# deepinv/deepinv

Hardware: AMD Instinct MI355X
Metric: PnP-PGD slices/sec (50 iters), 2D MRI 8-coil 320x320, 4x radial mask, DRUNet (higher is better)
Workload: dtype f32: fp32 multiplies and accumulation on the fp32 matrix cores (v_mfma_f32_32x32x2_f32); ResBlock convs as Winograd F(4x4,3x3), U = G g G^T formed in fp64 and rounded once; the three 2x2 stride-2 down convolutions (2 % of the FLOPs) as an exact three-part bf16 operand split with six products and fp3

## Files before the change

### deepinv_amd/csrc/drunet_bf16s.hip

```cpp
#include "drunet_common.hpp"

using namespace dinv;
using namespace dinv_drunet;

namespace {

__device__ __forceinline__ unsigned f2bf(float f) {
#ifdef DINV_EMU
    unsigned u = __float_as_uint(f);
    if ((u & 0x7fffffffu) > 0x7f800000u) return (u >> 16) | 0x40u;
    u += 0x7fffu + ((u >> 16) & 1u);
    return u >> 16;
#else
    return (unsigned)__builtin_bit_cast(unsigned short, (__bf16)f);
#endif
}
__device__ __forceinline__ float bf2f(unsigned h) { return __uint_as_float(h << 16); }

__device__ __forceinline__ void split8(const float4& a, const float4& b, uint4& hi, uint4& lo) {
    const float v[8] = {a.x, a.y, a.z, a.w, b.x, b.y, b.z, b.w};
    unsigned h[8], l[8];
#pragma unroll
    for (int e = 0; e < 8; ++e) {
        h[e] = f2bf(v[e]);
        l[e] = f2bf(v[e] - bf2f(h[e]));
    }
    hi = make_uint4(h[0] | (h[1] << 16), h[2] | (h[3] << 16), h[4] | (h[5] << 16), h[6] | (h[7] << 16));
    lo = make_uint4(l[0] | (l[1] << 16), l[2] | (l[3] << 16), l[4] | (l[5] << 16), l[6] | (l[7] << 16));
}

__device__ __forceinline__ void split8x3(const float4& a, const float4& b, uint4& hi, uint4& mi, uint4& lo) {
    const float v[8] = {a.x, a.y, a.z, a.w, b.x, b.y, b.z, b.w};
    unsigned h[8], m[8], l[8];
#pragma unroll
    for (int e = 0; e < 8; ++e) {
        h[e] = f2bf(v[e]);
        const float r1 = v[e] - bf2f(h[e]);
        m[e] = f2bf(r1);
        l[e] = f2bf(r1 - bf2f(m[e]));
    }
    hi = make_uint4(h[0] | (h[1] << 16), h[2] | (h[3] << 16), h[4] | (h[5] << 16), h[6] | (h[7] << 16));
    mi = make_uint4(m[0] | (m[1] << 16), m[2] | (m[3] << 16), m[4] | (m[5] << 16), m[6] | (m[7] << 16));
    lo = make_uint4(l[0] | (l[1] << 16), l[2] | (l[3] << 16), l[4] | (l[5] << 16), l[6] | (l[7] << 16));
}

#ifdef DINV_EMU
__device__ __forceinline__ f32x16 mfma_bf16(const uint4& a, const uint4& b, const f32x16& c) {
    emu_bf16x8 av, bv;
    std::memcpy(&av, &a, 16);
    std::memcpy(&bv, &b, 16);
    return emu_mfma_f32_32x32x16_bf16(av, bv, c);
}
#else
typedef __bf16 bf16x8 __attribute__((ext_vector_type(8)));
__device__ __forceinline__ f32x16 mfma_bf16(const uint4& a, const uint4& b, const f32x16& c) {
    return __builtin_amdgcn_mfma_f32_32x32x16_bf16(__builtin_bit_cast(bf16x8, a), __builtin_bit_cast(bf16x8, b), c, 0, 0, 0);
}
#endif

struct DownSArgs {
    Geom gi, go;
    const float* x;
    const uint4* w;
    float* y;
    int32_t cin, cout;
    int64_t ntiles, per_xcd;
    DepthMap dm;
};

template <bool ACC, int NPL>
__global__ __launch_bounds__(256) void down2x2_bf16s_kernel(DownSArgs a) {
    constexpr int WU = NPL * 128;
    constexpr int WPT = (WU + 255) / 256;
    __shared__ uint4 wl[2][WU];
    const int tid = threadIdx.x, lane = tid & 63, wv = tid >> 6;
    const int l31 = lane & 31, lhi = lane >> 5;
    const int64_t logical = (int64_t)(blockIdx.x & 7) * a.per_xcd + (blockIdx.x >> 3);
    if (logical >= a.ntiles) return;
    const int nct = a.cout / 64;
    const int64_t q0 = (logical / nct) * 256 + wv * 64;
    const int co0 = (int)(logical % nct) * 64;
    int64_t ioff[2];
    bool in[2];
#pragma unroll
    for (int n = 0; n < 2; ++n) {
        const int64_t q = q0 + n * 32 + l31;
        in[n] = interior(a.go, q);
        ioff[n] = a.gi.sl;
        if (in[n]) {
            const int64_t b = q / a.go.plane;
            const int64_t bi = depth_pair(a.dm, b);
            if (bi < 0) in[n] = false;
            else {
                const int qi = (int)(q - b * a.go.plane);
                const int R = qi / a.go.wp, C = qi - R * a.go.wp;
                ioff[n] = a.gi.sl + bi * a.gi.plane + (int64_t)(2 * (R - 1) + 1) * a.gi.wp + (2 * (C - 1) + 1);
            }
        }
    }
    f32x16 acc[2][2];
#pragma unroll
    for (int m = 0; m < 2; ++m)
#pragma unroll
        for (int n = 0; n < 2; ++n)
#pragma unroll
            for (int r = 0; r < 16; ++r) acc[m][n][r] = 0.f;
    const int S = a.cin / 16, nsteps = 4 * S;
    float4 ba[2], bb[2];
    uint4 wreg[WPT];
    auto issue = [&](int g) {
        const int tap = g / S, s = g - tap * S;
        const int64_t toff = (int64_t)(tap >> 1) * a.gi.wp + (tap & 1);
#pragma unroll
        for (int k = 0; k < WPT; ++k) {
            const int u = tid + 256 * k;
            if (u < WU) wreg[k] = a.w[((int64_t)g * (2 * NPL) + (u >> 6)) * a.cout + co0 + (u & 63)];
        }
#pragma unroll
        for (int n = 0; n < 2; ++n) {
            const float* xb = a.x + ((int64_t)(2 * s + lhi) * a.gi.cs + ioff[n] + toff) * 8;
            ba[n] = ld4(xb);
            bb[n] = ld4(xb + 4);
        }
    };
    uint4 Bp[NPL][2];
    auto commit = [&](int stage) {
#pragma unroll
        for (int k = 0; k < WPT; ++k)
            if (tid + 256 * k < WU) wl[stage][tid + 256 * k] = wreg[k];
#pragma unroll
        for (int n = 0; n < 2; ++n) {
            if constexpr (NPL == 2) split8(ba[n], bb[n], Bp[0][n], Bp[1][n]);
            else split8x3(ba[n], bb[n], Bp[0][n], Bp[1][n], Bp[2][n]);
        }
    };
    issue(0);
    commit(0);
    if (nsteps > 1) issue(1);
    __syncthreads();
    constexpr int NPROD = NPL == 2 ? 3 : 6;
    constexpr int PA[6] = {0, 1, 0, 0, 1, 0}, PB2[3] = {1, 0, 0};
    constexpr int QA[6] = {1, 0, 2, 0, 1, 0}, QB[6] = {1, 2, 0, 1, 0, 0};
    for (int g = 0; g < nsteps; ++g) {
        const uint4* ws = wl[g & 1];
        uint4 A[NPL][2];
#pragma unroll
        for (int pl = 0; pl < NPL; ++pl)
#pragma unroll
            for (int m = 0; m < 2; ++m) A[pl][m] = ws[pl * 128 + lhi * 64 + m * 32 + l31];
#pragma unroll
        for (int e = 0; e < NPROD; ++e) {
            const int pa = NPL == 2 ? PA[e] : QA[e], pb = NPL == 2 ? PB2[e] : QB[e];
#pragma unroll
            for (int m = 0; m < 2; ++m)
#pragma unroll
                for (int n = 0; n < 2; ++n) acc[m][n] = mfma_bf16(A[pa][m], Bp[pb][n], acc[m][n]);
        }
        if (g + 1 < nsteps) {
            commit((g + 1) & 1);
            if (g + 2 < nsteps) issue(g + 2);
        }
        lds_barrier();
    }
#pragma unroll
    for (int n = 0; n < 2; ++n) {
        const int64_t q = q0 + n * 32 + l31;
        if (q >= a.go.np) continue;
        store_tile<2, false, ACC ? 1 : 0>(acc, n, a.go.sl + q, in[n], co0 / 8, a.cout / 8, a.go.cs, lhi, a.y, ACC ? a.y : nullptr,
                                          nullptr);
    }
}

struct UpSArgs {
    Geom gi, go;
    const float* x;
    const float* x2;
    const uint4* w;
    float* y;
    int32_t cin, cout;
    DepthMap dm;
};

#ifdef DINV_EMU
#define DINV_BF16S_UP_ATTR
#else
#define DINV_BF16S_UP_ATTR __attribute__((amdgpu_waves_per_eu(2, 2)))
#endif
template <bool SKIP>
__global__ __launch_bounds__(256) DINV_BF16S_UP_ATTR void up2x2_bf16s_kernel(UpSArgs a) {
    __shared__ uint4 wl[2][1024];
    const int tid = threadIdx.x, lane = tid & 63, wv = tid >> 6;
    const int l31 = lane & 31, lhi = lane >> 5;
    const int tp = wv & 1, pg = wv >> 1;
    const int co0 = blockIdx.y * 64;
    const int64_t p0 = (int64_t)blockIdx.x * 128 + pg * 64;
    int64_t ioff[2], ooff[2];
    bool in[2];
#pragma unroll
    for (int n = 0; n < 2; ++n) {
        const int64_t p = p0 + n * 32 + l31;
        in[n] = interior(a.gi, p);
        ioff[n] = a.gi.sl + (in[n] ? p : 0);
        ooff[n] = 0;
        if (in[n]) {
            const int64_t b = p / a.gi.plane;
            const int64_t bo = depth_pair(a.dm, b);
            if (bo < 0) in[n] = false;
            else {
                const int pi = (int)(p - b * a.gi.plane);
                const int r = pi / a.gi.wp, c = pi - r * a.gi.wp;
                ooff[n] = a.go.sl + bo * a.go.plane + (int64_t)(2 * (r - 1) + 1 + tp) * a.go.wp + (2 * (c - 1) + 1);
            }
        }
    }
    f32x16 acc[2][2][2];
#pragma unroll
    for (int t = 0; t < 2; ++t)
#pragma unroll
        for (int m = 0; m < 2; ++m)
#pragma unroll
            for (int n = 0; n < 2; ++n)
#pragma unroll
                for (int r = 0; r < 16; ++r) acc[t][m][n][r] = 0.f;
    const int S = a.cin / 16;
    float4 ba[2], bb[2];
    uint4 wreg[4];
    auto issue = [&](int s) {
#pragma unroll
        for (int k = 0; k < 4; ++k) {
            const int u = tid + 256 * k;
            wreg[k] = a.w[((int64_t)s * 16 + (u >> 6)) * a.cout + co0 + (u & 63)];
        }
#pragma unroll
        for (int n = 0; n < 2; ++n) {
            const int64_t o = ((int64_t)(2 * s + lhi) * a.gi.cs + ioff[n]) * 8;
            ba[n] = ld4(a.x + o);
            bb[n] = ld4(a.x + o + 4);
            if (SKIP) {
                ba[n] = add4(ba[n], ld4(a.x2 + o));
                bb[n] = add4(bb[n], ld4(a.x2 + o + 4));
            }
        }
    };
    auto commit = [&](int stage, uint4 (&Bh)[2], uint4 (&Bl)[2]) {
#pragma unroll
        for (int k = 0; k < 4; ++k) wl[stage][tid + 256 * k] = wreg[k];
        split8(ba[0], bb[0], Bh[0], Bl[0]);
        split8(ba[1], bb[1], Bh[1], Bl[1]);
    };
    uint4 Bh[2], Bl[2];
    issue(0);
    commit(0, Bh, Bl);
    if (S > 1) issue(1);
    __syncthreads();
    for (int s = 0; s < S; ++s) {
        const uint4* ws = wl[s & 1] + (tp * 2) * 256;
#pragma unroll
        for (int t = 0; t < 2; ++t) {
            uint4 A[2][2];
#pragma unroll
            for (int pl = 0; pl < 2; ++pl)
#pragma unroll
                for (int m = 0; m < 2; ++m) A[pl][m] = ws[t * 256 + pl * 128 + lhi * 64 + m * 32 + l31];
#pragma unroll
            for (int e = 0; e < 3; ++e) {
                const int pa = e == 1 ? 1 : 0;
#pragma unroll
                for (int m = 0; m < 2; ++m)
#pragma unroll
                    for (int n = 0; n < 2; ++n) acc[t][m][n] = mfma_bf16(A[pa][m], e == 0 ? Bl[n] : Bh[n], acc[t][m][n]);
            }
        }
        if (s + 1 < S) {
            commit((s + 1) & 1, Bh, Bl);
            if (s + 2 < S) issue(s + 2);
        }
        lds_barrier();
    }
#pragma unroll
    for (int n = 0; n < 2; ++n) {
        if (!in[n]) continue;
#pragma unroll
        for (int t = 0; t < 2; ++t)
#pragma unroll
            for (int m = 0; m < 2; ++m)
#pragma unroll
                for (int rj = 0; rj < 4; ++rj) {
                    const float4 v = make_float4(acc[t][m][n][4 * rj], acc[t][m][n][4 * rj + 1], acc[t][m][n][4 * rj + 2],
                                                 acc[t][m][n][4 * rj + 3]);
                    st4(a.y + ((int64_t)(co0 / 8 + m * 4 + rj) * a.go.cs + ooff[n] + t) * 8 + 4 * lhi, v);
                }
    }
}

}

static int down2x2_bf16s_launch(const dinv_act_geom* gin, const dinv_act_geom* gout, const float* x, const void* w_split,
                                int32_t cin, int32_t cout, float* y, DepthMap dm, int accumulate, dinv_stream_t stream,
                                int planes = 2) {
    if (int e = check_geom(gin)) return e;
    if (int e = check_geom(gout)) return e;
    DINV_REQUIRE(x && w_split && y, "null tensor pointer");
    DINV_REQUIRE(gin->height == 2 * gout->height && gin->width == 2 * gout->width, "down2x2 geometry mismatch");
    if (dm.dep_s == 0) DINV_REQUIRE(gin->batch == gout->batch, "down2x2 geometry mismatch");
    else
        DINV_REQUIRE(dm.dep_s >= 3 && dm.dep_l == 2 * (dm.dep_s - 2) + 2 && gout->batch % dm.dep_s == 0 &&
                     gin->batch / dm.dep_l == gout->batch / dm.dep_s && gin->batch % dm.dep_l == 0 && (dm.dz == 0 || dm.dz == 1),
                     "down2x2: bad depth pairing (%d, %d, %d)", dm.dep_s, dm.dep_l, dm.dz);
    DINV_REQUIRE(cin >= 16 && cin % 16 == 0 && cout % 64 == 0, "bf16-split down2x2 needs cin %% 16 == 0 and cout %% 64 == 0 (got %d,%d)", cin, cout);
    DownSArgs a{make_geom(*gin), make_geom(*gout), x, reinterpret_cast<const uint4*>(w_split), y, cin, cout, 0, 0, dm};
    a.ntiles = ceil_div(gout->np, 256) * (cout / 64);
    a.per_xcd = ceil_div(a.ntiles, 8);
    const dim3 grid((unsigned)(a.per_xcd * 8));
    hipStream_t st = reinterpret_cast<hipStream_t>(stream);
    if (planes == 3) hipLaunchKernelGGL((down2x2_bf16s_kernel<false, 3>), grid, dim3(256), 0, st, a);
    else if (accumulate) hipLaunchKernelGGL((down2x2_bf16s_kernel<true, 2>), grid, dim3(256), 0, st, a);
    else hipLaunchKernelGGL((down2x2_bf16s_kernel<false, 2>), grid, dim3(256), 0, st, a);
    DINV_CHECK_LAUNCH();
    return 0;
}

extern "C" int dinv_conv_down2x2_bf16s(const dinv_act_geom* gin, const dinv_act_geom* gout, const float* x,
                                       const void* w_split, int32_t cin, int32_t cout, float* y, dinv_stream_t stream) {
    return down2x2_bf16s_launch(gin, gout, x, w_split, cin, cout, y, DepthMap{0, 0, 0}, 0, stream);
}

extern "C" int dinv_conv_down2x2_bf16x3(const dinv_act_geom* gin, const dinv_act_geom* gout, const float* x,
                                        const void* w_split3, int32_t cin, int32_t cout, float* y, dinv_stream_t stream) {
    return down2x2_bf16s_launch(gin, gout, x, w_split3, cin, cout, y, DepthMap{0, 0, 0}, 0, stream, 3);
}

extern "C" int dinv_conv_down2x2_bf16s_3d(const dinv_act_geom* gin, const dinv_act_geom* gout, const float* x,
                                          const void* w_split, int32_t cin, int32_t cout, float* y, int32_t depth_out,
                                          int32_t dz, int32_t accumulate, dinv_stream_t stream) {
    DINV_REQUIRE(depth_out >= 1, "bad depth %d", depth_out);
    return down2x2_bf16s_launch(gin, gout, x, w_split, cin, cout, y, DepthMap{depth_out + 2, 2 * depth_out + 2, dz}, accumulate, stream);
}

static int up2x2_bf16s_launch(const dinv_act_geom* gin, const dinv_act_geom* gout, const float* x, const float* x2,
                              const void* w_split, int32_t cin, int32_t cout, float* y, DepthMap dm, dinv_stream_t stream) {
    if (int e = check_geom(gin)) return e;
    if (int e = check_geom(gout)) return e;
    DINV_REQUIRE(x && w_split && y, "null tensor pointer");
    DINV_REQUIRE(gout->height == 2 * gin->height && gout->width == 2 * gin->width, "up2x2 geometry mismatch");
    if (dm.dep_s == 0) DINV_REQUIRE(gin->batch == gout->batch, "up2x2 geometry mismatch");
    else
        DINV_REQUIRE(dm.dep_s >= 3 && dm.dep_l == 2 * (dm.dep_s - 2) + 2 && gin->batch % dm.dep_s == 0 &&
                     gout->batch % dm.dep_l == 0 && gout->batch / dm.dep_l == gin->batch / dm.dep_s && (dm.dz == 0 || dm.dz == 1),
                     "up2x2: bad depth pairing (%d, %d, %d)", dm.dep_s, dm.dep_l, dm.dz);
    DINV_REQUIRE(cin >= 16 && cin % 16 == 0 && cout % 64 == 0, "bf16-split up2x2 needs cin %% 16 == 0 and cout %% 64 == 0 (got %d,%d)", cin, cout);
    UpSArgs a{make_geom(*gin), make_geom(*gout), x, x2, reinterpret_cast<const uint4*>(w_split), y, cin, cout, dm};
    const dim3 grid((unsigned)ceil_div(gin->np, 128), (unsigned)(cout / 64));
    hipStream_t st = reinterpret_cast<hipStream_t>(stream);
    if (x2) hipLaunchKernelGGL(up2x2_bf16s_kernel<true>, grid, dim3(256), 0, st, a);
    else hipLaunchKernelGGL(up2x2_bf16s_kernel<false>, grid, dim3(256), 0, st, a);
    DINV_CHECK_LAUNCH();
    return 0;
}

extern "C" int dinv_conv_up2x2_bf16s(const dinv_act_geom* gin, const dinv_act_geom* gout, const float* x, const float* x2,
                                     const void* w_split, int32_t cin, int32_t cout, float* y, dinv_stream_t stream) {
    return up2x2_bf16s_launch(gin, gout, x, x2, w_split, cin, cout, y, DepthMap{0, 0, 0}, stream);
}

extern "C" int dinv_conv_up2x2_bf16s_3d(const dinv_act_geom* gin, const dinv_act_geom* gout, const float* x, const float* x2,
                                        const void* w_split, int32_t cin, int32_t cout, float* y, int32_t depth_in, int32_t dz,
                                        dinv_stream_t stream) {
    DINV_REQUIRE(depth_in >= 1, "bad depth %d", depth_in);
    return up2x2_bf16s_launch(gin, gout, x, x2, w_split, cin, cout, y, DepthMap{depth_in + 2, 2 * depth_in + 2, dz}, stream);
}
```

Before: 15.94.

## Restructure bf16-split down2x2 kernel: stage activations in LDS, stream weights from registers

The down-convolution kernel is reorganized so each block covers 128 output pixels and up to 256 output channels. The bf16-split input activations are built cooperatively once and shared through LDS, while each wave reads its own weight fragments directly from global memory into double-buffered registers. Before, every wave split its own activations and the weights went through LDS. The aim is more input reuse across output channels and fewer redundant split conversions. The costs are more register pressure (MW×4 accumulators), a launch that depends on cout, and idle waves when cout is not a multiple of 128.

New measurement: 15.99 (median of 6 runs). About the same (+0.3%).

```diff
diff --git a/deepinv_amd/csrc/drunet_bf16s.hip b/deepinv_amd/csrc/drunet_bf16s.hip
--- a/deepinv_amd/csrc/drunet_bf16s.hip
+++ b/deepinv_amd/csrc/drunet_bf16s.hip
@@ -63,111 +63,128 @@
     const float* x;
     const uint4* w;
     float* y;
-    int32_t cin, cout;
+    int32_t cin, cout, nct;
     int64_t ntiles, per_xcd;
     DepthMap dm;
 };
 
-template <bool ACC, int NPL>
+template <bool ACC, int NPL, int MW>
 __global__ __launch_bounds__(256) void down2x2_bf16s_kernel(DownSArgs a) {
-    constexpr int WU = NPL * 128;
-    constexpr int WPT = (WU + 255) / 256;
-    __shared__ uint4 wl[2][WU];
+    __shared__ uint4 bs[2][2 * NPL * 2 * 128];
+    __shared__ int inl[128];
     const int tid = threadIdx.x, lane = tid & 63, wv = tid >> 6;
     const int l31 = lane & 31, lhi = lane >> 5;
+    const int px = tid & 127, uu = tid >> 7;
     const int64_t logical = (int64_t)(blockIdx.x & 7) * a.per_xcd + (blockIdx.x >> 3);
     if (logical >= a.ntiles) return;
-    const int nct = a.cout / 64;
-    const int64_t q0 = (logical / nct) * 256 + wv * 64;
-    const int co0 = (int)(logical % nct) * 64;
-    int64_t ioff[2];
-    bool in[2];
-#pragma unroll
-    for (int n = 0; n < 2; ++n) {
-        const int64_t q = q0 + n * 32 + l31;
-        in[n] = interior(a.go, q);
-        ioff[n] = a.gi.sl;
-        if (in[n]) {
+    const int64_t q0 = (logical / a.nct) * 128;
+    const int co_w = (int)(logical % a.nct) * (MW * 128) + wv * (MW * 32);
+    const bool active = co_w < a.cout;
+    int64_t ioff = a.gi.sl;
+    {
+        const int64_t q = q0 + px;
+        bool in = interior(a.go, q);
+        if (in) {
             const int64_t b = q / a.go.plane;
             const int64_t bi = depth_pair(a.dm, b);
-            if (bi < 0) in[n] = false;
+            if (bi < 0) in = false;
             else {
                 const int qi = (int)(q - b * a.go.plane);
                 const int R = qi / a.go.wp, C = qi - R * a.go.wp;
-                ioff[n] = a.gi.sl + bi * a.gi.plane + (int64_t)(2 * (R - 1) + 1) * a.gi.wp + (2 * (C - 1) + 1);
-            }
-        }
-    }
-    f32x16 acc[2][2];
-#pragma unroll
-    for (int m = 0; m < 2; ++m)
-#pragma unroll
-        for (int n = 0; n < 2; ++n)
+                ioff = a.gi.sl + bi * a.gi.plane + (int64_t)(2 * (R - 1) + 1) * a.gi.wp + (2 * (C - 1) + 1);
+            }
+        }
+        if (uu == 0) inl[px] = in;
+    }
+    f32x16 acc[MW][4];
+#pragma unroll
+    for (int m = 0; m < MW; ++m)
+#pragma unroll
+        for (int n = 0; n < 4; ++n)
 #pragma unroll
             for (int r = 0; r < 16; ++r) acc[m][n][r] = 0.f;
-    const int S = a.cin / 16, nsteps = 4 * S;
-    float4 ba[2], bb[2];
-    uint4 wreg[WPT];
-    auto issue = [&](int g) {
-        const int tap = g / S, s = g - tap * S;
-        const int64_t toff = (int64_t)(tap >> 1) * a.gi.wp + (tap & 1);
-#pragma unroll
-        for (int k = 0; k < WPT; ++k) {
-            const int u = tid + 256 * k;
-            if (u < WU) wreg[k] = a.w[((int64_t)g * (2 * NPL) + (u >> 6)) * a.cout + co0 + (u & 63)];
-        }
-#pragma unroll
-        for (int n = 0; n < 2; ++n) {
-            const float* xb = a.x + ((int64_t)(2 * s + lhi) * a.gi.cs + ioff[n] + toff) * 8;
-            ba[n] = ld4(xb);
-            bb[n] = ld4(xb + 4);
-        }
-    };
-    uint4 Bp[NPL][2];
-    auto commit = [&](int stage) {
-#pragma unroll
-        for (int k = 0; k < WPT; ++k)
-            if (tid + 256 * k < WU) wl[stage][tid + 256 * k] = wreg[k];
-#pragma unroll
-        for (int n = 0; n < 2; ++n) {
-            if constexpr (NPL == 2) split8(ba[n], bb[n], Bp[0][n], Bp[1][n]);
-            else split8x3(ba[n], bb[n], Bp[0][n], Bp[1][n], Bp[2][n]);
-        }
-    };
-    issue(0);
-    commit(0);
-    if (nsteps > 1) issue(1);
-    __syncthreads();
+    const int CB = a.cin / 8, S = a.cin / 16, nst = CB;
+    float4 xr[4];
+    auto issueB = [&](int sg) {
+        const int u = 2 * sg + uu, dy = u >= CB ? 1 : 0, cb = u - dy * CB;
+        const float* xb = a.x + ((int64_t)cb * a.gi.cs + ioff + (int64_t)dy * a.gi.wp) * 8;
+#pragma unroll
+        for (int k = 0; k < 4; ++k) xr[k] = ld4(xb + 4 * k);
+    };
+    auto commitB = [&](int stage) {
+        uint4* dst = bs[stage] + uu * (NPL * 256) + px;
+#pragma unroll
+        for (int dx = 0; dx < 2; ++dx) {
+            uint4 P[NPL];
+            if constexpr (NPL == 2) split8(xr[2 * dx], xr[2 * dx + 1], P[0], P[1]);
+            else split8x3(xr[2 * dx], xr[2 * dx + 1], P[0], P[1], P[2]);
+#pragma unroll
+            for (int pl = 0; pl < NPL; ++pl) dst[(pl * 2 + dx) * 128] = P[pl];
+        }
+    };
+    auto issueA = [&](int u, uint4 (&A)[NPL][MW]) {
+        const int dy = u >= CB ? 1 : 0, cb = u - dy * CB;
+        const int64_t g = (int64_t)(dy * 2 + lhi) * S + (cb >> 1);
+        const uint4* wb = a.w + (g * (2 * NPL) + (cb & 1)) * a.cout + co_w + l31;
+#pragma unroll
+        for (int pl = 0; pl < NPL; ++pl)
+#pragma unroll
+            for (int m = 0; m < MW; ++m) A[pl][m] = wb[(int64_t)pl * 2 * a.cout + m * 32];
+    };
     constexpr int NPROD = NPL == 2 ? 3 : 6;
     constexpr int PA[6] = {0, 1, 0, 0, 1, 0}, PB2[3] = {1, 0, 0};
     constexpr int QA[6] = {1, 0, 2, 0, 1, 0}, QB[6] = {1, 2, 0, 1, 0, 0};
-    for (int g = 0; g < nsteps; ++g) {
-        const uint4* ws = wl[g & 1];
-        uint4 A[NPL][2];
+    auto step = [&](const uint4* bu, const uint4 (&A)[NPL][MW]) {
+        uint4 Bf[NPL][4];
 #pragma unroll
         for (int pl = 0; pl < NPL; ++pl)
 #pragma unroll
-            for (int m = 0; m < 2; ++m) A[pl][m] = ws[pl * 128 + lhi * 64 + m * 32 + l31];
+            for (int n = 0; n < 4; ++n) Bf[pl][n] = bu[(pl * 2 + lhi) * 128 + n * 32 + l31];
 #pragma unroll
         for (int e = 0; e < NPROD; ++e) {
             const int pa = NPL == 2 ? PA[e] : QA[e], pb = NPL == 2 ? PB2[e] : QB[e];
 #pragma unroll
-            for (int m = 0; m < 2; ++m)
-#pragma unroll
-                for (int n = 0; n < 2; ++n) acc[m][n] = mfma_bf16(A[pa][m], Bp[pb][n], acc[m][n]);
-        }
-        if (g + 1 < nsteps) {
-            commit((g + 1) & 1);
-            if (g + 2 < nsteps) issue(g + 2);
+            for (int m = 0; m < MW; ++m)
+#pragma unroll
+                for (int n = 0; n < 4; ++n) acc[m][n] = mfma_bf16(A[pa][m], Bf[pb][n], acc[m][n]);
+        }
+    };
+    uint4 A0[NPL][MW], A1[NPL][MW];
+    issueB(0);
+    if (active) issueA(0, A0);
+    commitB(0);
+    if (nst > 1) issueB(1);
+    __syncthreads();
+    for (int sg = 0; sg < nst; ++sg) {
+        const uint4* bst = bs[sg & 1];
+        if (active) {
+            issueA(2 * sg + 1, A1);
+            step(bst, A0);
+            if (sg + 1 < nst) issueA(2 * sg + 2, A0);
+            step(bst + NPL * 256, A1);
+        }
+        if (sg + 1 < nst) {
+            commitB((sg + 1) & 1);
+            if (sg + 2 < nst) issueB(sg + 2);
         }
         lds_barrier();
     }
-#pragma unroll
-    for (int n = 0; n < 2; ++n) {
+    if (!active) return;
+#pragma unroll
+    for (int n = 0; n < 4; ++n) {
         const int64_t q = q0 + n * 32 + l31;
         if (q >= a.go.np) continue;
-        store_tile<2, false, ACC ? 1 : 0>(acc, n, a.go.sl + q, in[n], co0 / 8, a.cout / 8, a.go.cs, lhi, a.y, ACC ? a.y : nullptr,
-                                          nullptr);
+        const bool in = inl[n * 32 + l31] != 0;
+#pragma unroll
+        for (int m = 0; m < MW; ++m)
+#pragma unroll
+            for (int g = 0; g < 4; ++g) {
+                float* yp = a.y + ((int64_t)(co_w / 8 + 4 * m + g) * a.go.cs + a.go.sl + q) * 8 + 4 * lhi;
+                float4 v = make_float4(acc[m][n][4 * g], acc[m][n][4 * g + 1], acc[m][n][4 * g + 2], acc[m][n][4 * g + 3]);
+                if (ACC) v = add4(v, ld4(yp));
+                if (!in) v = make_float4(0.f, 0.f, 0.f, 0.f);
+                st4(yp, v);
+            }
     }
 }
 
@@ -308,14 +325,22 @@
                      gin->batch / dm.dep_l == gout->batch / dm.dep_s && gin->batch % dm.dep_l == 0 && (dm.dz == 0 || dm.dz == 1),
                      "down2x2: bad depth pairing (%d, %d, %d)", dm.dep_s, dm.dep_l, dm.dz);
     DINV_REQUIRE(cin >= 16 && cin % 16 == 0 && cout % 64 == 0, "bf16-split down2x2 needs cin %% 16 == 0 and cout %% 64 == 0 (got %d,%d)", cin, cout);
-    DownSArgs a{make_geom(*gin), make_geom(*gout), x, reinterpret_cast<const uint4*>(w_split), y, cin, cout, 0, 0, dm};
-    a.ntiles = ceil_div(gout->np, 256) * (cout / 64);
+    const int mw = cout % 256 == 0 ? 2 : 1;
+    const int nct = (int)ceil_div(cout, mw * 128);
+    DownSArgs a{make_geom(*gin), make_geom(*gout), x, reinterpret_cast<const uint4*>(w_split), y, cin, cout, nct, 0, 0, dm};
+    a.ntiles = ceil_div(gout->np, 128) * nct;
     a.per_xcd = ceil_div(a.ntiles, 8);
     const dim3 grid((unsigned)(a.per_xcd * 8));
     hipStream_t st = reinterpret_cast<hipStream_t>(stream);
-    if (planes == 3) hipLaunchKernelGGL((down2x2_bf16s_kernel<false, 3>), grid, dim3(256), 0, st, a);
-    else if (accumulate) hipLaunchKernelGGL((down2x2_bf16s_kernel<true, 2>), grid, dim3(256), 0, st, a);
-    else hipLaunchKernelGGL((down2x2_bf16s_kernel<false, 2>), grid, dim3(256), 0, st, a);
+#define DINV_DOWN_LAUNCH(ACC, NPL)                                                                             \
+    do {                                                                                                       \
+        if (mw == 2) hipLaunchKernelGGL((down2x2_bf16s_kernel<ACC, NPL, 2>), grid, dim3(256), 0, st, a);       \
+        else hipLaunchKernelGGL((down2x2_bf16s_kernel<ACC, NPL, 1>), grid, dim3(256), 0, st, a);               \
+    } while (0)
+    if (planes == 3) DINV_DOWN_LAUNCH(false, 3);
+    else if (accumulate) DINV_DOWN_LAUNCH(true, 2);
+    else DINV_DOWN_LAUNCH(false, 2);
+#undef DINV_DOWN_LAUNCH
     DINV_CHECK_LAUNCH();
     return 0;
 }
```
